# bwvdnbro/CMacIonize

Measured on AMD Instinct MI355X. Metric: photon packets/sec, 256^3 stromgren, higher is better.
Workload: dtype f64

## Files before the change

### cmacionize_amd/csrc/engine.hip

```cpp
#include "../../include/cmi_gpu.h"

#include "atomic_data.h"
#include "linecooling_data.h"
#include "kernels.h"
#include "dust_kernels.h"
#include "line_image_kernels.h"
#include "line_cube_kernels.h"
#include "sky_image_kernels.h"
#include "sky_cube_kernels.h"
#include "dust_cube_kernels.h"
#include "continuum_kernels.h"
#include "absorbing_cube_kernels.h"
#include "lyman_alpha_kernels.h"
#include "absorption_kernels.h"
#include "sort.h"

#include <algorithm>
#include <climits>
#include <cmath>
#include <cstdarg>
#include <cstdlib>
#include <cstdio>
#include <cstring>
#include <new>
// ... 102 lines not shown
  uint64_t tile_capacity = 0;
  bool tile_has_weights = false;
  FlightRowsDev tile_rows[2];
  uint32_t *tile_iota = nullptr;
  TileItemDev *tile_items = nullptr;
  uint32_t *tile_begin = nullptr;
  uint32_t *tile_blockhist = nullptr, *tile_total = nullptr;
  uint32_t *tile_new_slots = nullptr;
  TrackersDev trackers = {};
  bool trackers_enabled = false;
  EscapeDev escape = {};
  bool escape_counting = false;
  EscapeDev escape_staged = {};
  double *pad_H = nullptr;
  bool pad_valid = false;
  unsigned long long *metal_gate = nullptr;
  bool metals_pending = false;
  bool state_pointer_escaped = false;
  char *temp_pipe_block = nullptr;
  uint32_t temp_pipe_capacity = 0;
  unsigned int *temp_pipe_counts = nullptr;
  uint32_t *tile_ended_slot = nullptr;
  uint32_t *tile_ended_pos = nullptr;
  uint32_t *tile_slot_of[2] = {nullptr, nullptr};
  unsigned int *tile_absorbed_count = nullptr;
  unsigned int *tile_absorbed_before = nullptr;
  unsigned int *tile_counts = nullptr;
  uint64_t tile_rounds_run = 0;
  bool acc_block_dirty = false;

// ... 13 lines not shown
    bool reemit_passes = true;
    int refill_threshold_reemit = 32;
    int64_t reemit_inline_below = -1;
    int reemit_max_passes = 12;
    bool tile_rounds = true;
    uint64_t tile_min_flights = 100000;
    int tile_min_per_item = -1;
    int tile_refill_threshold = 48;
    bool tile_counting_sort = true;
    bool update_reuse = true;
    bool defer_metals = true;
    bool update_writes_pad = true;
    bool defer_weights = true;
    bool pre_emission = true;
    bool pad_march = true;
    bool xcd_remap = false;
    bool temperature_pipeline = true;
    uint32_t temperature_finish_slots = 1024;
    int tile_compact_ratio = -1;
    bool park_in_place = true;
    bool span_claim = CMI_SPAN_CLAIM_DEFAULT;
    bool emit_before_flush = CMI_EMIT_BEFORE_FLUSH_DEFAULT;
    bool phase_stamps = false;
    int continuum_channel_block = CMI_CONTINUUM_FB;
    int64_t continuum_launch_rays = 0;
    int absorbing_cube_channel_block = CMI_ABSORBING_CB;
    int absorbing_cube_expm1_call = CMI_ABSORBING_EXPM1_CALL;
    int absorbing_cube_window_skip = 1;
    int64_t absorbing_cube_launch_rays = 0;
    int absorption_slab_rows = 0;
// ... 606 lines not shown
  for (int64_t i = (int64_t)blockIdx.x * blockDim.x + threadIdx.x; i < n;
       i += step)
    dst[i * stride] = src[i];
}

int grid_blocks(cmi_gpu_engine *e, int64_t work_items, int blocks_per_cu) {
  int64_t want = (work_items + CMI_BLOCK - 1) / CMI_BLOCK;
  int64_t cap = (int64_t)e->num_cu * blocks_per_cu;
  if (want < 1)
    want = 1;
  return (int)(want < cap ? want : cap);
}

int update_full_flag(cmi_gpu_engine *e) {
  bool full = e->model.xsec_verner != 0;
  if (!full)
    for (int i = 1; i < CMI_NION; ++i)
      if (e->model.xsec_fixed[i] != 0.)
        full = true;
  if (full != e->full_ions)
    CMI_TRY(settle_metal_fractions(e));
  if (full != e->full_ions && e->acc_block) {
    if (hipSetDevice(e->device) != hipSuccess ||
        hipMemsetAsync(e->acc_block, 0,
                       (size_t)CMI_NACC * e->ncell * sizeof(double),
                       e->stream) != hipSuccess)
      e->acc_block_dirty = true;
  }
  e->full_ions = full;
  CellsDev &cells = cells_of_iteration(e);
// ... 724 lines not shown
  return field_pointer(e, field);
}

int cmi_gpu_get_update_state(cmi_gpu_engine *e, int32_t *metals_pending,
                             int32_t *pad_records_valid,
                             int32_t *deferral_allowed) {
  if (!e)
    return fail(CMI_GPU_EINVAL, "null engine");
  if (metals_pending)
    *metals_pending = e->metals_pending ? 1 : 0;
  if (pad_records_valid)
    *pad_records_valid = e->pad_valid ? 1 : 0;
  if (deferral_allowed)
    *deferral_allowed =
        (e->tune.defer_metals && !e->state_pointer_escaped) ? 1 : 0;
  return CMI_GPU_OK;
}

int cmi_gpu_reset_grid(cmi_gpu_engine *e) {
  if (!e)
    return fail(CMI_GPU_EINVAL, "null engine");
  HIP_TRY(hipSetDevice(e->device));
  const size_t field_bytes = (size_t)e->ncell * sizeof(double);
  if (e->full_ions || e->acc_block_dirty) {
    HIP_TRY(hipMemsetAsync(e->acc_block, 0, CMI_NACC * field_bytes,
                           e->stream));
    e->acc_block_dirty = false;
  } else {
    HIP_TRY(hipMemsetAsync(e->acc_block, 0, field_bytes, e->stream));
    if (e->config.track_heating)
// ... 55 lines not shown
  else if (k == "tile_refill_threshold")
    e->tune.tile_refill_threshold =
        (int)(value < 1 ? 1 : (value > 64 ? 64 : value));
  else if (k == "tile_compact_ratio")
    e->tune.tile_compact_ratio = (int)(value < -1 ? -1 : value);
  else if (k == "park_in_place")
    e->tune.park_in_place = value != 0;
  else if (k == "accumulators_dirty")
    e->acc_block_dirty = e->acc_block_dirty || value != 0;
  else if (k == "temperature_finish_slots")
    e->tune.temperature_finish_slots = (uint32_t)(value < 0 ? 0 : value);
  else if (k == "temperature_pipeline")
    e->tune.temperature_pipeline = value != 0;
  else if (k == "pad_march")
    e->tune.pad_march = value != 0;
  else if (k == "xcd_remap")
    e->tune.xcd_remap = value != 0;
  else if (k == "pre_emission")
    e->tune.pre_emission = value != 0;
  else if (k == "defer_weights")
    e->tune.defer_weights = value != 0;
  else if (k == "tile_counting_sort")
    e->tune.tile_counting_sort = value != 0;
  else if (k == "update_reuse")
    e->tune.update_reuse = value != 0;
  else if (k == "defer_metals")
    e->tune.defer_metals = value != 0;
  else if (k == "update_writes_pad")
    e->tune.update_writes_pad = value != 0;
  else if (k == "span_claim")
// ... 335 lines not shown
  const double volume =
      e->grid.cellside[0] * e->grid.cellside[1] * e->grid.cellside[2];
  a.jfac = jfac / volume;
  a.hfac = hfac / volume;
  a.first = first_cell;
  a.count = ncell;

  EventPair ev;
  CMI_TRY(timer_begin(e, ev));
  const int blocks = grid_blocks(e, ncell, 8);
  if (defer) {
    HydrogenUpdateArgs h;
    h.u = a;
    h.gate = e->metal_gate;
    h.pad_H = (e->pad_valid && e->tune.update_writes_pad) ? e->pad_H : nullptr;
    h.ny = (uint32_t)e->grid.ncell[1];
    h.nz = (uint32_t)e->grid.ncell[2];
    if (!h.pad_H)
      pad_records_stale(e);
    if (e->config.track_heating)
      hydrogen_update_kernel<true><<<blocks, CMI_BLOCK, 0, e->stream>>>(h);
    else
      hydrogen_update_kernel<false><<<blocks, CMI_BLOCK, 0, e->stream>>>(h);
    HIP_TRY(hipGetLastError());
    e->metals_pending = true;
    CMI_TRY(timer_end(e, e->update_events, ev, 0));
    return CMI_GPU_OK;
  }
  pad_records_stale(e);
  if (solve_temperature && e->tune.temperature_pipeline) {
// ... 736 lines not shown
```

### cmacionize_amd/csrc/kernels.h

```cpp
#ifndef CMI_KERNELS_H
#define CMI_KERNELS_H

#include "device_transport.h"
#include "device_reemit.h"
#include "device_thermal.h"
#include "device_emissivity.h"

#ifndef CMI_BLOCK
#define CMI_BLOCK 256
#endif
#ifdef CMI_EXPERIMENTS
#define CMI_EXP(a) ((a).exp_no_atomics)
#else
#define CMI_EXP(a) 0
#endif
#ifndef CMI_TABLE_BITS
#define CMI_TABLE_BITS 10
#endif
#define CMI_TABLE_SLOTS (1 << CMI_TABLE_BITS)
#ifndef CMI_TABLE_BLOCK
#define CMI_TABLE_BLOCK 512
#endif
#ifndef CMI_TABLE_BLOCK_BITS
#define CMI_TABLE_BLOCK_BITS 11
// ... 98 lines not shown
  uint32_t seed;
  uint32_t iteration;
  int32_t refill_threshold;
  int32_t exp_no_atomics;
  TrackersDev trackers;
  int32_t aggregate;
  QueueDev qin, qout;
  int32_t park_in_place;
  const double *xin;
  int32_t xin_local;
#ifdef CMI_DBG_XIN_SLOTS
  const uint32_t *xin_slots = nullptr;
#endif
  ExchangeDev xout;
  const double *pad_H;
  int32_t xcd_remap;
  int32_t pad_ny, pad_nz;
  double pad_inv_yz, pad_inv_z;
  uint32_t *span_cursor;
  uint32_t n_spans;
  int32_t span_claim;
  int32_t emit_before_flush;
#ifdef CMI_EXPERIMENTS
  unsigned long long *phase_clock;
#endif
};

#define CMI_SPAN_WANTED 0xfffffffeu
#define CMI_SPAN_NONE 0xffffffffu
#define CMI_SPAN_CURSORS 8
// ... 7 lines not shown
  CMI_PHASE_COUNT
};

#ifndef CMI_FULL_WAVES
#define CMI_FULL_WAVES 4
#endif
#ifndef CMI_PAD_WAVES
#define CMI_PAD_WAVES 8
#endif
#ifndef CMI_PAD_SCAN_ROUNDS
#define CMI_PAD_SCAN_ROUNDS 3
#endif
#define CMI_PAD_LAYERS 1
#define CMI_PAD_VACUUM (-0.)
#define CMI_PAD_GHOST (-2.)
__device__ __forceinline__ int32_t cmi_pad_index(int32_t offset) {
  return (int32_t)((uint32_t)offset >> 3);
}
__device__ __forceinline__ int32_t cmi_unpad_cell(const ShootArgs &a,
                                                  const GridDev &g,
                                                  int32_t c) {
  const double cc = (double)c + 0.5;
  const int32_t ix = (int32_t)(cc * a.pad_inv_yz);
  const int32_t r = c - ix * (a.pad_ny * a.pad_nz);
  const int32_t iy = (int32_t)(((double)r + 0.5) * a.pad_inv_z);
  const int32_t iz = r - iy * a.pad_nz;
  return ((ix - CMI_PAD_LAYERS) * g.ncell[1] + (iy - CMI_PAD_LAYERS)) *
             g.ncell[2] +
         (iz - CMI_PAD_LAYERS);
}
// ... 594 lines not shown
    const int32_t gi = p.index[ax] + g.offset[ax];
    in_block &= (p.index[ax] >= 0 && p.index[ax] < g.ncell[ax]);
    in_grid &= (gi >= 0 && gi < g.global_ncell[ax]);
  }
  const bool at_origin = (g.offset[0] | g.offset[1] | g.offset[2]) == 0;
  bool mine = in_block || (!in_grid && at_origin);
  if (g.copy_count > 1)
    mine &= (int32_t)(packet_id % (uint32_t)g.copy_count) == g.copy_rank;
  return mine;
}

#ifndef CMI_FULL_PASS_WAVES
#define CMI_FULL_PASS_WAVES 3
#endif
template <bool FULL, bool HEAT, bool REEMIT, bool EXACT, bool TABLE = false,
          bool PRE = false, bool PAD = false, bool TRACK = false,
          bool BIG = false>
__global__ void
    __launch_bounds__((shoot_block_threads<FULL, TABLE, BIG>()),
                      REEMIT ? 1
                             : (FULL ? (TABLE ? CMI_FULL_WAVES
                                              : CMI_FULL_PASS_WAVES)
                                    : ((PAD && !HEAT) ? CMI_PAD_WAVES
                                       : BIG          ? 4
                                                      : 6)))
        shoot_kernel(const ShootArgs a) {
  static_assert(!BIG || PAD, "BIG: the padded march on large grids");
  constexpr int BLOCK = shoot_block_threads<FULL, TABLE, BIG>();
  constexpr int TBITS =
      (TABLE && !FULL)
          ? (BIG ? CMI_TABLE_BLOCK_BIG_BITS : CMI_TABLE_BLOCK_BITS)
          : CMI_TABLE_BITS;
  constexpr int TSLOTS = 1 << TBITS;
  static_assert(!PAD || (TABLE && !FULL && !REEMIT && !EXACT && !PRE),
                "PAD is a specialisation of the hydrogen-only TABLE kernel");
  static_assert(!TRACK || (!TABLE && !EXACT && !PRE && !PAD),
                "TRACK is the tracker hook in the plain incremental marcher");
  const int lane = threadIdx.x & 63;
  const uint64_t lane_lt = (1ull << lane) - 1ull;
  uint32_t block = blockIdx.x;
  if (a.xcd_remap) {
    const uint32_t xcd = block & 7u, q = gridDim.x >> 3, r = gridDim.x & 7u;
    block = (xcd < r ? xcd * (q + 1u) : r * (q + 1u) + (xcd - r) * q) +
            (block >> 3);
  }
  const uint64_t wave = (uint64_t)block * (BLOCK / 64) +
                        (threadIdx.x >> 6);
  const uint64_t nwaves = (uint64_t)gridDim.x * (BLOCK / 64);
  const uint64_t chunk = a.chunk;

  uint64_t chunk_begin = wave * chunk;
  uint64_t pos = chunk_begin;
// ... 142 lines not shown
            atomic_add_f64(a.cells.acc_base + (int64_t)t * CMI_NACC + i,
                           lds_val[k * CMI_NACC + i]);
            lds_val[k * CMI_NACC + i] = 0.;
            ++natomics;
          }
          if (i == 0)
            lds_tag[k] = -1;
        }
      }
    } else {
      for (int k = threadIdx.x; k < lds_slots; k += BLOCK) {
        const int32_t t = lds_tag[TS * k];
        if (PAD ? t != -1 : t >= 0) {
          const int32_t c =
              PAD ? cmi_unpad_cell(a, a.grid, cmi_pad_index(t)) : t;
          atomic_add_f64(acc_at(a.cells, ION_H_n, c), lds_val[k]);
          lds_val[k] = 0.;
          if (HEAT) {
            atomic_add_f64(acc_at(a.cells, CMI_NION, c),
                           lds_val[lds_slots + k]);
            lds_val[lds_slots + k] = 0.;
          }
          lds_tag[TS * k] = -1;
          natomics += HEAT ? 2 : 1;
        }
      }
    }
    int any_work = 0, all_waves = 2;
#pragma unroll
    for (int w = 0; w < BLOCK / 64; ++w) {
      any_work |= block_has_work[w];
// ... 68 lines not shown
      }
      if (lanes_of(found)) {
        atomicAdd(&lds_val[slot], v0);
        if (HEAT)
          atomicAdd(&lds_val[TSLOTS + slot], v1);
      }
      looking &= ~found;
      if (lanes_of(looking))
        slot = (slot + 1) & (TSLOTS - 1);
      if (looking == 0ull)
        return;
    }
    if (lanes_of(looking)) {
      const int32_t c =
          PAD ? cmi_unpad_cell(a, a.grid, cmi_pad_index(cell)) : cell;
      atomic_add_f64(acc_at(a.cells, ION_H_n, c), v0);
      if (HEAT)
        atomic_add_f64(acc_at(a.cells, CMI_NION, c), v1);
      natomics += HEAT ? 2 : 1;
    }
  };
  for (;;) {
    const unsigned long long active_mask = __ballot(active);
    const unsigned long long idle_mask = ~active_mask;
    if (!claim && pos == pos_end &&
        chunk_begin + nwaves * chunk < a.n_packets) {
      chunk_begin += nwaves * chunk;
      pos = chunk_begin;
      pos_end = chunk_begin + chunk < a.n_packets ? chunk_begin + chunk
                                                  : a.n_packets;
    }
// ... 147 lines not shown
      }
      const uint64_t taken = __popcll(idle_mask);
      pos += taken < avail ? taken : avail;
    }
    CMI_PHASE_MARK(CMI_PHASE_REFILL);
    if (CLAIM && refill_first && !flush_point(has_work))
      break;
    const uint64_t avail_after =
        (pos_end - pos) +
        (!claim && chunk_begin + nwaves * chunk < a.n_packets ? 1 : 0);

    int window = 0;
    if (FULL)
      load_quarter_weights(stage, wq);
    if constexpr (PAD) {
      const double sigma = p.sigma_H;
      double wsig = p.weight * p.sigma_H;
      double hw = HEAT ? wsig * (p.nu - a.model.nu_H) : 0.;
      asm volatile("" : "+v"(wsig), "+v"(hw));
      const unsigned long long active_lanes = wave_ballot(active);
      int32_t not_lane = ~(lane << 3);
      asm volatile("" : "+v"(not_lane));
      const __attribute__((address_space(1))) char *pad_base =
          (const __attribute__((address_space(1))) char *)a.pad_H;
      asm volatile("" : "+s"(pad_base));
      const int idle_limit = __builtin_amdgcn_readfirstlane(
          avail_after != 0 ? a.refill_threshold : 65);
      const int fly_min = idle_limit < 64 ? 64 - idle_limit : 0;
      int zero = 0;
      asm volatile("" : "+v"(zero));
      const RunMasks pad_run_masks = run_masks<CMI_PAD_SCAN_ROUNDS>();
      unsigned int bundle_steps = 0;
      unsigned int bundle_lane_steps = 0;
      unsigned long long in_flight = active_lanes & mask_gt(p.tau, 0.);
      unsigned long long flying = in_flight & mask_gt(pad_next, -1.5);
      int nflying = (int)__popcll(flying);
      if (nflying > fly_min) do {
        ++bundle_steps;
        bundle_lane_steps += (unsigned int)nflying;
        const bool stepping = lanes_of(flying);
        const unsigned long long accumulating =
            flying & mask_ge(__double2hiint(pad_next), 0);
        int32_t key = lanes_of(accumulating) ? p.cell : not_lane;
        asm volatile("" : "+v"(key));
        double ds;
        asm volatile("" : "=v"(ds));
        if (stepping) {
          const double tmin =
              min_f64(p.tmax[0], min_f64(p.tmax[1], p.tmax[2]));
          const double t_old = p.t;
          ds = tmin - t_old;
          const double sk = sigma * pad_next;
          p.tau -= ds * sk;
          {
            unsigned long long saved;
            asm volatile("s_and_saveexec_b64 %[saved], %[m0]\n\t"
                         "v_add_f64 %[t0], %[t0], %[d0]\n\t"
                         "v_add_u32 %[cell], %[cell], %[c0]\n\t"
                         "s_and_b64 exec, %[saved], %[m1]\n\t"
                         "v_add_f64 %[t1], %[t1], %[d1]\n\t"
                         "v_add_u32 %[cell], %[cell], %[c1]\n\t"
                         "s_and_b64 exec, %[saved], %[m2]\n\t"
                         "v_add_f64 %[t2], %[t2], %[d2]\n\t"
                         "v_add_u32 %[cell], %[cell], %[c2]\n\t"
                         "s_mov_b64 exec, %[saved]"
                         : [t0] "+v"(p.tmax[0]), [t1] "+v"(p.tmax[1]),
                           [t2] "+v"(p.tmax[2]), [cell] "+v"(p.cell),
// ... 15 lines not shown
              double corr = p.tau * r;
              corr = __fma_rn(__fma_rn(-corr, sk, p.tau), r, corr);
              ds += corr;
              p.t = t_old + ds;
            }
          }
          pad_next = *reinterpret_cast<
              const __attribute__((address_space(1))) double *>(
              pad_base + (uint32_t)p.cell);
        }
        in_flight = flying & mask_gt(p.tau, 0.);
        if (CMI_EXP(a) == 12) {
          asm volatile("" ::"v"(ds), "s"(accumulating));
          continue;
        }
        double v[2] = {ds * wsig, HEAT ? ds * hw : 0.};
        unsigned long long tails;
        if (HEAT)
          run_sums_masked<2, CMI_PAD_SCAN_ROUNDS>(key, v, tails, zero,
                                                  pad_run_masks);
        else
          run_sums_masked<1, CMI_PAD_SCAN_ROUNDS>(
              key, reinterpret_cast<double(&)[1]>(v), tails, zero,
              pad_run_masks);
        if (CMI_EXP(a) == 11) {
          asm volatile("" ::"v"(v[0]), "s"(tails));
          continue;
        }
        table_add_masked(tails & accumulating, key, v[0], v[1]);
      } while ((flying = in_flight & mask_gt(pad_next, -1.5),
                nflying = (int)__popcll(flying), nflying > fly_min));
// ... 1297 lines not shown
      if (use_stored) {
        const MetalTermsStored terms = {&stored};
        ionization_update_cell<HEATING>(a, c, ntot, T, J, heating, terms);
      } else {
        const MetalTermsEvaluated terms = {a.model, T, T * 1.e-4};
        ionization_update_cell<HEATING>(a, c, ntot, T, J, heating, terms);
      }
    }
  }
}

struct HydrogenUpdateArgs {
  UpdateArgs u;
  unsigned long long *gate;
  double *pad_H;
  uint32_t ny, nz;
};

#ifndef CMI_HYDROGEN_UPDATE_WAVES
#define CMI_HYDROGEN_UPDATE_WAVES 4
#endif
template <bool HEATING>
__global__ void __launch_bounds__(CMI_BLOCK, CMI_HYDROGEN_UPDATE_WAVES)
    hydrogen_update_kernel(const HydrogenUpdateArgs h) {
  constexpr int WAVES = CMI_BLOCK / 64;
  const UpdateArgs &a = h.u;
  const int64_t rows = (a.count + 63) >> 6;
  const int64_t nwaves = (int64_t)gridDim.x * WAVES;
  const uint32_t lane = threadIdx.x & 63u;
  for (int64_t row = (int64_t)blockIdx.x * WAVES + (threadIdx.x >> 6);
// ... 15 lines not shown
      a.cells.x[ION_He_n][c] = he0;
      if (HEATING) {
        (*acc_at(a.cells, CMI_NION, c)) = heating[0];
        (*acc_at(a.cells, CMI_NION + 1, c)) = heating[1];
      }
      const double2 k = (ntot > 0.) ? make_double2(ntot * h0, ntot * he0)
                                    : make_double2(-1., 0.);
      a.cells.opacity[c] = k;
      if (h.pad_H) {
        constexpr uint32_t L = CMI_PAD_LAYERS;
        const uint32_t cc = (uint32_t)c;
        const uint32_t xy = cc / h.nz, pz = cc - xy * h.nz;
        const uint32_t px = xy / h.ny, py = xy - px * h.ny;
        const uint32_t padded =
            ((px + L) * (h.ny + 2 * L) + (py + L)) * (h.nz + 2 * L) + pz + L;
        h.pad_H[padded] = (k.x >= 0.) ? k.x : CMI_PAD_VACUUM;
      }
    }
    const unsigned long long word = wave_ballot(gate);
    if (lane == 0)
      h.gate[row] = word;
  }
}

struct MetalFractionsArgs {
  ModelDev model;
  CellsDev cells;
  int64_t count;
  const unsigned long long *gate;
};

// ... 277 lines not shown
__global__ void __launch_bounds__(CMI_BLOCK)
    opacity_kernel(const CellsDev cells, int64_t ncell) {
  const int64_t stride = (int64_t)gridDim.x * blockDim.x;
  for (int64_t c = (int64_t)blockIdx.x * blockDim.x + threadIdx.x; c < ncell;
       c += stride) {
    const double ntot = cells.number_density[c];
    cells.opacity[c] =
        (ntot > 0.) ? make_double2(ntot * cells.x[ION_H_n][c],
                                   ntot * cells.x[ION_He_n][c])
                    : make_double2(-1., 0.);
  }
}

__global__ void __launch_bounds__(CMI_BLOCK)
    pad_record_kernel(const double2 *__restrict__ opacity, double *pad,
                      int32_t nx, int32_t ny, int32_t nz) {
  const int64_t total = (int64_t)(nx + 2 * CMI_PAD_LAYERS) *
                        (ny + 2 * CMI_PAD_LAYERS) * (nz + 2 * CMI_PAD_LAYERS);
  const int64_t stride = (int64_t)gridDim.x * blockDim.x;
  for (int64_t c = (int64_t)blockIdx.x * blockDim.x + threadIdx.x; c < total;
       c += stride) {
    constexpr int L = CMI_PAD_LAYERS;
    const int32_t pz = (int32_t)(c % (nz + 2 * L)) - L;
    const int32_t py = (int32_t)((c / (nz + 2 * L)) % (ny + 2 * L)) - L;
    const int32_t px = (int32_t)(c / ((int64_t)(nz + 2 * L) * (ny + 2 * L))) - L;
    double v = CMI_PAD_GHOST;
    if (px >= 0 && px < nx && py >= 0 && py < ny && pz >= 0 && pz < nz) {
      const double k = opacity[((int64_t)px * ny + py) * nz + pz].x;
      v = (k >= 0.) ? k : CMI_PAD_VACUUM;
    }
    pad[c] = v;
  }
}


__global__ void emit_probe_kernel(const GridDev grid, const ModelDev model,
                                  uint32_t seed, uint32_t iteration,
                                  uint64_t first, uint64_t n, double *position,
                                  double *direction, double *frequency,
                                  double *sigma, double *tau) {
  const uint64_t i = (uint64_t)blockIdx.x * blockDim.x + threadIdx.x;
  if (i >= n)
    return;
  PacketRng rng;
  rng.init(seed, iteration, first + i);
// ... 72 lines not shown
```

### cmacionize_amd/csrc/transport_driver.h

```cpp
#ifndef CMI_TRANSPORT_DRIVER_H
#define CMI_TRANSPORT_DRIVER_H

static int reserve_sort_buffers(cmi_gpu_engine *e, uint64_t n) {
  if (e->sort_capacity >= n)
    return CMI_GPU_OK;
  HIP_TRY(hipStreamSynchronize(e->stream));
  (void)hipFree(e->sort_keys[0]);
  (void)hipFree(e->sort_temp);
  e->sort_keys[0] = nullptr;
  e->sort_temp = nullptr;
  e->sort_capacity = 0;
  uint32_t *block = nullptr;
  HIP_TRY(hipMalloc(&block, sizeof(uint32_t) * 4 * n));
  e->sort_keys[0] = block;
  e->sort_keys[1] = block + n;
  e->sort_ids[0] = block + 2 * n;
  e->sort_ids[1] = block + 3 * n;
  size_t bytes = 0;
  HIP_TRY(cmi_sort_pairs_temp_bytes(n, 32, &bytes));
  e->sort_temp_bytes = bytes;
  HIP_TRY(hipMalloc(&e->sort_temp, bytes ? bytes : 16));
  e->sort_capacity = n;
  return CMI_GPU_OK;
}
// ... 169 lines not shown
  FIRST_PAD_BIG,
  FIRST_PRE
};

struct LaunchPlan {
  bool heat, reemit;
  bool exact;
  bool tracking;
  bool passes;
  bool tiles;
  bool sorted;
  bool select_mode;
  int agg, agg_reemit;
  FirstBuild first;
  bool pad, pad_big;
  int64_t padded_cells;
  ShootKernel kernel, kernel_inline, kernel_first;
  int blocks_per_cu, blocks_per_cu_inline, blocks_per_cu_first;
  int first_threads;
  uint32_t tau_bits, source_bits, dir_bits;
  int key_bits;
  double sigma_ref;
  TileKernel tile_kernel;
  int tile_threads, tile_blocks_per_cu;
};

static ShootKernel shoot_build(bool full, bool heat, bool reemit, bool exact,
                               bool track, FirstBuild first) {
  static const ShootKernel generic[2][4][2] = {
      {{shoot_kernel<false, false, false, false>,
        shoot_kernel<false, false, true, false>},
       {shoot_kernel<false, true, false, false>,
        shoot_kernel<false, true, true, false>},
       {shoot_kernel<true, false, false, false>,
        shoot_kernel<true, false, true, false>},
       {shoot_kernel<true, true, false, false>,
        shoot_kernel<true, true, true, false>}},
      {{shoot_kernel<false, false, false, true>,
        shoot_kernel<false, false, true, true>},
       {shoot_kernel<false, true, false, true>,
        shoot_kernel<false, true, true, true>},
       {shoot_kernel<true, false, false, true>,
        shoot_kernel<true, false, true, true>},
// ... 1 lines not shown
        shoot_kernel<true, true, true, true>}}};
  static const ShootKernel tracked[4][2] = {
      {shoot_kernel<false, false, false, false, false, false, false, true>,
       shoot_kernel<false, false, true, false, false, false, false, true>},
      {shoot_kernel<false, true, false, false, false, false, false, true>,
       shoot_kernel<false, true, true, false, false, false, false, true>},
      {shoot_kernel<true, false, false, false, false, false, false, true>,
       shoot_kernel<true, false, true, false, false, false, false, true>},
      {shoot_kernel<true, true, false, false, false, false, false, true>,
       shoot_kernel<true, true, true, false, false, false, false, true>}};
  static const ShootKernel table[2][2] = {
      {shoot_kernel<true, true, false, false, true>,
       shoot_kernel<true, false, false, false, true>},
      {shoot_kernel<false, true, false, false, true>,
       shoot_kernel<false, false, false, false, true>}};
  static const ShootKernel pad_big[2] = {
      shoot_kernel<false, true, false, false, true, false, true, false, true>,
      shoot_kernel<false, false, false, false, true, false, true, false, true>};
  static const ShootKernel pad[2] = {
      shoot_kernel<false, true, false, false, true, false, true>,
      shoot_kernel<false, false, false, false, true, false, true>};
  static const ShootKernel pre[2] = {
      shoot_kernel<true, true, false, false, true, true>,
      shoot_kernel<true, false, false, false, true, true>};
  switch (first) {
  case FIRST_TABLE:
    return table[!full][!heat];
  case FIRST_PAD:
    return pad[!heat];
  case FIRST_PAD_BIG:
    return pad_big[!heat];
  case FIRST_PRE:
    return pre[!heat];
  case FIRST_GENERIC:
    break;
  }
  return track ? tracked[2 * full + heat][reemit]
               : generic[exact][2 * full + heat][reemit];
}

extern "C++" {
template <class Kernel>
static int blocks_per_cu_of(Kernel kernel, int threads, int most, int &out) {
  out = 0;
  HIP_TRY(hipOccupancyMaxActiveBlocksPerMultiprocessor(&out, kernel, threads,
                                                       0));
// ... 18 lines not shown
  p.exact = tune.exact_dda || !small_grid ||
            (p.tracking && !e->grid.decomposed);
  p.passes = p.reemit && tune.reemit_passes &&
             !(flights && n_packets < reemit_inline_below(e));
  p.sorted = tune.sort_packets && !flights;
  p.tiles = p.passes && tune.tile_rounds && !p.exact && !p.tracking;
  p.select_mode = p.sorted && e->grid.decomposed;

  const bool table =
      !flights && !p.exact && !p.tracking && p.agg == CMI_AGG_BLOCK &&
      (p.passes || !p.reemit) &&
      !(e->grid.periodic[0] | e->grid.periodic[1] | e->grid.periodic[2]);
  p.padded_cells = ((int64_t)e->grid.ncell[0] + 2 * CMI_PAD_LAYERS) *
                   ((int64_t)e->grid.ncell[1] + 2 * CMI_PAD_LAYERS) *
                   ((int64_t)e->grid.ncell[2] + 2 * CMI_PAD_LAYERS);
  p.pad = table && !e->full_ions && tune.pad_march &&
          p.padded_cells < ((int64_t)1 << 29);
  p.pad_big = p.pad && e->ncell > CMI_TABLE_BIG_CELLS;
  p.first = FIRST_GENERIC;
  if (p.pad)
    p.first = p.pad_big ? FIRST_PAD_BIG : FIRST_PAD;
  else if (table && e->full_ions && tune.pre_emission && p.sorted &&
           p.tiles)
    p.first = FIRST_PRE;
  else if (table)
    p.first = FIRST_TABLE;
  p.first_threads = (table && !e->full_ions)
                        ? (p.pad_big ? shoot_block_threads<false, true, true>()
                                     : shoot_block_threads<false, true>())
                        : CMI_BLOCK;

  const bool track = p.tracking && !p.exact;
  p.kernel_inline =
      shoot_build(e->full_ions, p.heat, true, p.exact, track, FIRST_GENERIC);
  p.kernel = (p.reemit && !p.passes)
                 ? p.kernel_inline
                 : shoot_build(e->full_ions, p.heat, false, p.exact, track,
                               FIRST_GENERIC);
  p.kernel_first = table ? shoot_build(e->full_ions, p.heat, false, false,
                                       false, p.first)
                         : p.kernel;
  CMI_TRY(blocks_per_cu_of(p.kernel, CMI_BLOCK, tune.max_blocks_per_cu,
                           p.blocks_per_cu));
  CMI_TRY(blocks_per_cu_of(p.kernel_inline, CMI_BLOCK, tune.max_blocks_per_cu,
                           p.blocks_per_cu_inline));
  p.blocks_per_cu_first = p.blocks_per_cu;
  if (table)
    CMI_TRY(blocks_per_cu_of(p.kernel_first, p.first_threads,
                             tune.max_blocks_per_cu, p.blocks_per_cu_first));
  p.tile_kernel = nullptr;
  p.tile_threads = p.tile_blocks_per_cu = 0;
  if (p.tiles) {
    if (e->full_ions)
      p.tile_kernel =
          p.heat ? tile_kernel<true, true> : tile_kernel<true, false>;
// ... 98 lines not shown
  a.grid = e->grid;
  a.model = e->model;
  a.cells = cells_of_iteration(e);
  a.counters = e->counters;
  a.first_packet = first_packet;
  a.batch_offset = done;
  a.n_packets = nids;
  a.order = nullptr;
  a.pre_rows = nullptr;
  a.xin = flights ? flights + (size_t)CMI_FLIGHT_DOUBLES * done : nullptr;
  a.xin_local = 0;
  a.xout.rows = e->export_rows;
  a.xout.count = e->export_count;
  a.xout.capacity = (unsigned int)e->export_capacity;
  a.pad_H = p.pad ? e->pad_H : nullptr;
  a.xcd_remap = (p.sorted && e->tune.xcd_remap) ? 1 : 0;
  a.pad_ny = e->grid.ncell[1] + 2 * CMI_PAD_LAYERS;
  a.pad_nz = e->grid.ncell[2] + 2 * CMI_PAD_LAYERS;
  a.pad_inv_yz = 1. / ((double)a.pad_ny * (double)a.pad_nz);
  a.pad_inv_z = 1. / (double)a.pad_nz;
  a.chunk = e->tune.chunk;
  a.seed = seed;
  a.iteration = iteration;
  a.refill_threshold = flights ? e->tune.refill_threshold_reemit
                               : e->tune.refill_threshold;
  a.exp_no_atomics = e->tune.exp_no_atomics;
  a.trackers = e->trackers;
  if (!p.tracking)
    a.trackers.n = 0;
  a.aggregate = flights ? p.agg_reemit : p.agg;
// ... 6 lines not shown
  a.emit_before_flush = e->tune.emit_before_flush ? 1 : 0;
#ifdef CMI_EXPERIMENTS
  a.phase_clock = nullptr;
#endif
  return a;
}

static int pad_records(cmi_gpu_engine *e, const LaunchPlan &p) {
  if (e->pad_valid)
    return CMI_GPU_OK;
  const GridDev &g = e->grid;
  if (!e->pad_H)
    HIP_TRY(hipMalloc(&e->pad_H, sizeof(double) * (size_t)p.padded_cells));
  pad_record_kernel<<<grid_blocks(e, p.padded_cells, 8), CMI_BLOCK, 0,
                      e->stream>>>(cells_of_iteration(e).opacity, e->pad_H,
                                   g.ncell[0], g.ncell[1], g.ncell[2]);
  HIP_TRY(hipGetLastError());
  e->pad_valid = true;
  return CMI_GPU_OK;
}

static int select_block_packets(cmi_gpu_engine *e, ShootArgs &a,
                                const uint32_t **select) {
  const uint64_t nids = a.n_packets;
  if (!e->select_count)
    HIP_TRY(hipMalloc(&e->select_count, sizeof(unsigned int)));
  CMI_TRY(grow(e, e->select_ids, e->select_capacity, nids,
               sizeof(uint32_t) * nids));
  HIP_TRY(hipMemsetAsync(e->select_count, 0, sizeof(unsigned int),
                         e->stream));
  SelectArgs sa;
// ... 477 lines not shown
                "cmi_gpu_shoot: at most 2^32 - 2 packets per call");
  if (e->grid.decomposed &&
      (e->tune.exact_dda || !e->export_rows ||
       e->ncell >= CMI_FAST_MARCHER_MAX_CELLS))
    return fail(CMI_GPU_ESTATE,
                "cmi_gpu_shoot: a block of a decomposed grid needs an export "
                "buffer (cmi_gpu_set_export_buffer) and the incremental "
                "marcher (fewer than 2^28 cells per block)");
  if (!flights && e->grid.decomposed && block_emits_nothing(e))
    return CMI_GPU_OK;
  HIP_TRY(hipSetDevice(e->device));
  CMI_TRY(ensure_spectra(e));

  LaunchPlan plan;
  CMI_TRY(plan_launches(e, n_packets, flights, plan));
  CMI_TRY(publish_escape(e, plan.tracking));
  const uint64_t max_launch = e->tune.max_packets_per_launch;
  if (!plan.select_mode)
    CMI_TRY(reserve_for(e, plan, n_packets < max_launch ? n_packets
                                                         : max_launch));
  if (plan.pad)
    CMI_TRY(pad_records(e, plan));

  for (uint64_t done = 0; done < n_packets; done += max_launch) {
    const uint64_t nids = n_packets - done < max_launch ? n_packets - done
                                                        : max_launch;
    ShootArgs a = shoot_args(e, plan, seed, iteration, first_packet, done,
                             nids, flights);
    const uint32_t *select = nullptr;
    if (plan.select_mode) {
// ... 25 lines not shown
```

### cmacionize_amd/engine.py

```python
import ctypes as C
import os

import numpy as np

_HERE = os.path.dirname(os.path.abspath(__file__))
LIB_PATH = os.environ.get("CMI_GPU_LIBRARY",
                          os.path.join(_HERE, "libcmi_gpu.so"))

NION = 14
TRACKER_SPECTRUM, TRACKER_ABSORPTION, TRACKER_WEIGHTED_SPECTRUM = 0, 1, 2
NACC = 16
NTYPE = 4

FIELD_NUMBER_DENSITY = 0
FIELD_TEMPERATURE = 1
FIELD_IONIC_FRACTION = 2
FIELD_MEAN_INTENSITY = 16
FIELD_HEATING = 30

REEMIT_NONE, REEMIT_PHYSICAL, REEMIT_FIXED = 0, 1, 2
CONTINUOUS_NONE, CONTINUOUS_ISOTROPIC, CONTINUOUS_PLANAR = 0, 1, 2
ROLE_SOURCE, ROLE_CONTINUOUS = 0, 1
TABLE_LINEAR, TABLE_LOGLOG = 0, 1
DUST_PROBE_EMIT, DUST_PROBE_SCATTER, DUST_PROBE_SCATTER_TOWARDS = 0, 1, 2
# ... 100 lines not shown
    "cmi_gpu_render_continuum_sky_map", "cmi_gpu_continuum_probe",
    "cmi_gpu_hi_coefficients", "cmi_gpu_render_hi_cube",
    "cmi_gpu_render_hi_sky_cube", "cmi_gpu_render_hi_sky_map_cube",
    "cmi_gpu_render_field_absorbing_cube",
    "cmi_gpu_render_field_absorbing_sky_cube",
    "cmi_gpu_absorbing_cube_probe", "cmi_gpu_get_update_state",
    "cmi_gpu_set_lyman_alpha", "cmi_gpu_lya_shoot", "cmi_gpu_lya_probe",
    "cmi_gpu_download_lya_view", "cmi_gpu_reset_lya",
    "cmi_gpu_get_lya_counters", "cmi_gpu_lyman_alpha_emissivity",
    "cmi_gpu_set_lya_field", "cmi_gpu_download_lya_field",
    "cmi_gpu_lya_spin_temperature",
    "cmi_gpu_render_field_absorption_spectra",
    "cmi_gpu_render_absorption_spectra", "cmi_gpu_absorption_probe",
    "cmi_gpu_set_escape_tally", "cmi_gpu_reset_escape_tally",
    "cmi_gpu_download_escape_tally", "cmi_gpu_escape_pixels",
    "cmi_gpu_cross_sections",
]

EMISSION_LINES = [
    "HAlpha", "HBeta", "HII", "BALMER_JUMP_LOW", "BALMER_JUMP_HIGH",
    "OI_6300", "OI_6364", "OII_3727", "OIII_5007", "OIII_4959", "OIII_4363",
    "OIII_52mu", "OIII_88mu", "NII_5755", "NII_6548", "NII_6584",
    "NeIII_3869", "NeIII_3968", "SII_6725", "SII_4072", "SIII_9405",
    "SIII_6312", "SIII_19mu", "SIII_33mu", "avg_T", "avg_T_count",
    "avg_nH_nHe", "avg_nH_nHe_count", "NeII_12mu", "NIII_57mu", "NeIII_15mu",
    "NII_122mu", "CII_158mu", "CII_2325", "CIII_1908", "OII_7325", "SIV_10mu",
    "HeI_5876", "Hrec_s", "WFC2_F439W", "WFC2_F555W", "WFC2_F675W"]

_ELEMENT_WEIGHTS = {"H": 1.00794, "He": 4.002602, "C": 12.0107, "N": 14.0067,
                    "O": 15.9994, "Ne": 20.1797, "S": 32.065}

# ... 131 lines not shown
    L.cmi_gpu_set_cross_sections_verner.argtypes = [vp]
    L.cmi_gpu_set_recombination_rates_fixed.argtypes = [vp, _dp]
    L.cmi_gpu_set_recombination_rates_verner.argtypes = [vp]
    L.cmi_gpu_set_abundances.argtypes = [vp, _dp]
    L.cmi_gpu_set_reemission.argtypes = [vp, C.c_int32, C.c_double,
                                         C.c_double]
    L.cmi_gpu_set_temperature_params.argtypes = [
        vp, C.POINTER(TemperatureParams)]
    L.cmi_gpu_upload_cells.argtypes = [vp, _dp, _dp, _dp]
    L.cmi_gpu_upload_field.argtypes = [vp, C.c_int32, _dp]
    L.cmi_gpu_download_field.argtypes = [vp, C.c_int32, _dp]
    L.cmi_gpu_field_device_pointer.restype = C.c_void_p
    L.cmi_gpu_field_device_pointer.argtypes = [vp, C.c_int32]
    if hasattr(L, "cmi_gpu_get_update_state"):
        L.cmi_gpu_get_update_state.argtypes = [vp] + 3 * [C.POINTER(C.c_int32)]
    L.cmi_gpu_reset_grid.argtypes = [vp]
    L.cmi_gpu_shoot.argtypes = [vp, C.c_uint32, C.c_uint32, C.c_uint64,
                                C.c_uint64]
    L.cmi_gpu_get_counters.argtypes = [vp, _dp, _dp, C.POINTER(C.c_uint64)]
    L.cmi_gpu_update_cells.argtypes = [vp, C.c_uint32, C.c_double]
    L.cmi_gpu_emit_packets.argtypes = [vp, C.c_uint32, C.c_uint32, C.c_uint64,
                                       C.c_uint64, _dp, _dp, _dp, _dp, _dp]
    L.cmi_gpu_trace_packets.argtypes = [
        vp, C.c_uint64, _dp, _dp, _dp, _dp, _dp, C.c_int32,
        C.POINTER(C.c_int64), _dp, C.POINTER(C.c_int32), C.POINTER(C.c_int64),
        _dp]
    L.cmi_gpu_get_timing.argtypes = [vp, C.c_int32, _dp, C.POINTER(C.c_uint64),
                                     _dp, C.POINTER(C.c_uint64)]
    L.cmi_gpu_get_kernel_timing.argtypes = [vp, _dp, C.POINTER(C.c_uint64)]
    L.cmi_gpu_set_tuning.argtypes = [vp, C.c_char_p, C.c_int64]
# ... 582 lines not shown
    def accumulator_layout(self):
        fs, cs = C.c_int64(), C.c_int64()
        self._check(self._lib.cmi_gpu_accumulator_layout(
            self._h, C.byref(fs), C.byref(cs)))
        return fs.value, cs.value

    def field_device_pointer(self, field):
        return self._lib.cmi_gpu_field_device_pointer(self._h, field)

    def update_state(self):
        v = [C.c_int32() for _ in range(3)]
        self._check(self._lib.cmi_gpu_get_update_state(
            self._h, *[C.byref(x) for x in v]))
        return tuple(bool(x.value) for x in v)

    def field_tensor(self, field):
        import torch
        ptr = self.field_device_pointer(field)
        n = self.n

        class _View:
            __cuda_array_interface__ = {
                "shape": (n,), "typestr": "<f8", "data": (int(ptr), False),
                "version": 2}
        return torch.as_tensor(_View(), device="cuda")

    def refresh_transport_records(self):
        self._check(self._lib.cmi_gpu_refresh_transport_records(self._h))

    def reset_grid(self):
# ... 1186 lines not shown
```

### include/cmi_gpu.h

```cpp
#ifndef CMI_GPU_H
#define CMI_GPU_H

#include <stddef.h>
#include <stdint.h>

#ifdef __cplusplus
extern "C" {
#endif

#define CMI_GPU_NION 14
#define CMI_GPU_NHEATING 2
#define CMI_GPU_NTYPE 4
#define CMI_GPU_NACC (CMI_GPU_NION + CMI_GPU_NHEATING)

enum {
  CMI_GPU_OK = 0,
  CMI_GPU_EINVAL = 1,
  CMI_GPU_EDEVICE = 2,
  CMI_GPU_ESTATE = 3,
  CMI_GPU_ENOMEM = 4
};

enum {
  CMI_GPU_FIELD_NUMBER_DENSITY = 0,
// ... 102 lines not shown
int cmi_gpu_set_temperature_params(cmi_gpu_engine *engine,
                                   const cmi_gpu_temperature_params *params);


int cmi_gpu_upload_cells(cmi_gpu_engine *engine, const double *number_density,
                         const double *temperature,
                         const double *ionic_fractions);
int cmi_gpu_upload_field(cmi_gpu_engine *engine, int32_t field,
                         const double *values);
int cmi_gpu_download_field(cmi_gpu_engine *engine, int32_t field,
                           double *values);
void *cmi_gpu_field_device_pointer(cmi_gpu_engine *engine, int32_t field);
int cmi_gpu_get_update_state(cmi_gpu_engine *engine, int32_t *metals_pending,
                             int32_t *pad_records_valid,
                             int32_t *deferral_allowed);
int cmi_gpu_accumulator_layout(cmi_gpu_engine *engine, int64_t *field_stride,
                               int64_t *cell_stride);


int cmi_gpu_reset_grid(cmi_gpu_engine *engine);

int cmi_gpu_shoot(cmi_gpu_engine *engine, uint32_t seed, uint32_t iteration,
                  uint64_t first_packet, uint64_t n_packets);

#define CMI_GPU_FLIGHT_DOUBLES 16
int cmi_gpu_set_export_buffer(cmi_gpu_engine *engine, void *device_rows,
                              uint64_t capacity);
int cmi_gpu_get_export_count(cmi_gpu_engine *engine, uint64_t *count);
int cmi_gpu_reset_exports(cmi_gpu_engine *engine);
int cmi_gpu_download_exports(cmi_gpu_engine *engine, double *host_rows,
// ... 480 lines not shown
```

Measured before the change: 4.005 billion.

## Pre-multiply hydrogen cross-section into pad records and add uniform-weight PAD kernel

Pad records now store sigma_H times opacity, so the marcher's per-step multiply by sigma goes away. When packet weights are uniform and heating is off, a new specialised PAD kernel accumulates raw path lengths and applies a single weight times sigma scale at the atomic flush, removing a per-packet multiply and a register. Pad validity is now reset whenever the cross-section setup may change. The change also adds a query API reporting the chosen plan, and it rounds products differently than before.

```diff
diff --git a/cmacionize_amd/csrc/engine.hip b/cmacionize_amd/csrc/engine.hip
--- a/cmacionize_amd/csrc/engine.hip
+++ b/cmacionize_amd/csrc/engine.hip
@@ -140,6 +140,8 @@
   EscapeDev escape_staged = {};
   double *pad_H = nullptr;
   bool pad_valid = false;
+  int32_t last_first_build = 0;
+  bool last_pad_uniform = false;
   unsigned long long *metal_gate = nullptr;
   bool metals_pending = false;
   bool state_pointer_escaped = false;
@@ -183,6 +185,7 @@
     bool defer_weights = true;
     bool pre_emission = true;
     bool pad_march = true;
+    bool pad_uniform = true;
     bool xcd_remap = false;
     bool temperature_pipeline = true;
     uint32_t temperature_finish_slots = 1024;
@@ -819,6 +822,7 @@
 
 int update_full_flag(cmi_gpu_engine *e) {
   bool full = e->model.xsec_verner != 0;
+  e->pad_valid = false;
   if (!full)
     for (int i = 1; i < CMI_NION; ++i)
       if (e->model.xsec_fixed[i] != 0.)
@@ -1573,6 +1577,17 @@
   if (deferral_allowed)
     *deferral_allowed =
         (e->tune.defer_metals && !e->state_pointer_escaped) ? 1 : 0;
+  return CMI_GPU_OK;
+}
+
+int cmi_gpu_get_transport_plan(cmi_gpu_engine *e, int32_t *first_build,
+                               int32_t *uniform_weight) {
+  if (!e)
+    return fail(CMI_GPU_EINVAL, "null engine");
+  if (first_build)
+    *first_build = e->last_first_build;
+  if (uniform_weight)
+    *uniform_weight = e->last_pad_uniform ? 1 : 0;
   return CMI_GPU_OK;
 }
 
@@ -1658,6 +1673,8 @@
     e->tune.temperature_pipeline = value != 0;
   else if (k == "pad_march")
     e->tune.pad_march = value != 0;
+  else if (k == "pad_uniform")
+    e->tune.pad_uniform = value != 0;
   else if (k == "xcd_remap")
     e->tune.xcd_remap = value != 0;
   else if (k == "pre_emission")
@@ -2023,6 +2040,7 @@
     h.u = a;
     h.gate = e->metal_gate;
     h.pad_H = (e->pad_valid && e->tune.update_writes_pad) ? e->pad_H : nullptr;
+    h.pad_sigma = e->model.xsec_fixed[ION_H_n];
     h.ny = (uint32_t)e->grid.ncell[1];
     h.nz = (uint32_t)e->grid.ncell[2];
     if (!h.pad_H)
diff --git a/cmacionize_amd/csrc/kernels.h b/cmacionize_amd/csrc/kernels.h
--- a/cmacionize_amd/csrc/kernels.h
+++ b/cmacionize_amd/csrc/kernels.h
@@ -136,6 +136,7 @@
 #endif
   ExchangeDev xout;
   const double *pad_H;
+  double uniform_scale;
   int32_t xcd_remap;
   int32_t pad_ny, pad_nz;
   double pad_inv_yz, pad_inv_z;
@@ -173,6 +174,9 @@
 #define CMI_PAD_LAYERS 1
 #define CMI_PAD_VACUUM (-0.)
 #define CMI_PAD_GHOST (-2.)
+__device__ __forceinline__ double cmi_pad_record(double sigma, double nx) {
+  return sigma * ((nx >= 0.) ? nx : CMI_PAD_VACUUM);
+}
 __device__ __forceinline__ int32_t cmi_pad_index(int32_t offset) {
   return (int32_t)((uint32_t)offset >> 3);
 }
@@ -797,7 +801,7 @@
 #define CMI_FULL_PASS_WAVES 3
 #endif
 template <bool FULL, bool HEAT, bool REEMIT, bool EXACT, bool TABLE = false,
-          bool PRE = false, bool PAD = false, bool TRACK = false,
+          bool PRE = false, bool PAD = false, bool SWITCH8 = false,
           bool BIG = false>
 __global__ void
     __launch_bounds__((shoot_block_threads<FULL, TABLE, BIG>()),
@@ -817,8 +821,12 @@
   constexpr int TSLOTS = 1 << TBITS;
   static_assert(!PAD || (TABLE && !FULL && !REEMIT && !EXACT && !PRE),
                 "PAD is a specialisation of the hydrogen-only TABLE kernel");
-  static_assert(!TRACK || (!TABLE && !EXACT && !PRE && !PAD),
+  constexpr bool TRACK = SWITCH8 && !PAD;
+  static_assert(!TRACK || (!TABLE && !EXACT && !PRE),
                 "TRACK is the tracker hook in the plain incremental marcher");
+  constexpr bool UNIFORM = SWITCH8 && PAD;
+  static_assert(!UNIFORM || !HEAT,
+                "the heating term's weight differs from packet to packet");
   const int lane = threadIdx.x & 63;
   const uint64_t lane_lt = (1ull << lane) - 1ull;
   uint32_t block = blockIdx.x;
@@ -991,7 +999,8 @@
         if (PAD ? t != -1 : t >= 0) {
           const int32_t c =
               PAD ? cmi_unpad_cell(a, a.grid, cmi_pad_index(t)) : t;
-          atomic_add_f64(acc_at(a.cells, ION_H_n, c), lds_val[k]);
+          atomic_add_f64(acc_at(a.cells, ION_H_n, c),
+                         UNIFORM ? lds_val[k] * a.uniform_scale : lds_val[k]);
           lds_val[k] = 0.;
           if (HEAT) {
             atomic_add_f64(acc_at(a.cells, CMI_NION, c),
@@ -1090,7 +1099,8 @@
     if (lanes_of(looking)) {
       const int32_t c =
           PAD ? cmi_unpad_cell(a, a.grid, cmi_pad_index(cell)) : cell;
-      atomic_add_f64(acc_at(a.cells, ION_H_n, c), v0);
+      atomic_add_f64(acc_at(a.cells, ION_H_n, c),
+                     UNIFORM ? v0 * a.uniform_scale : v0);
       if (HEAT)
         atomic_add_f64(acc_at(a.cells, CMI_NION, c), v1);
       natomics += HEAT ? 2 : 1;
@@ -1268,10 +1278,10 @@
     if (FULL)
       load_quarter_weights(stage, wq);
     if constexpr (PAD) {
-      const double sigma = p.sigma_H;
-      double wsig = p.weight * p.sigma_H;
+      double wsig = UNIFORM ? 0. : p.weight * p.sigma_H;
       double hw = HEAT ? wsig * (p.nu - a.model.nu_H) : 0.;
-      asm volatile("" : "+v"(wsig), "+v"(hw));
+      if (!UNIFORM)
+        asm volatile("" : "+v"(wsig), "+v"(hw));
       const unsigned long long active_lanes = wave_ballot(active);
       int32_t not_lane = ~(lane << 3);
       asm volatile("" : "+v"(not_lane));
@@ -1295,16 +1305,16 @@
         const bool stepping = lanes_of(flying);
         const unsigned long long accumulating =
             flying & mask_ge(__double2hiint(pad_next), 0);
+        double t12 = min_f64(p.tmax[1], p.tmax[2]);
         int32_t key = lanes_of(accumulating) ? p.cell : not_lane;
-        asm volatile("" : "+v"(key));
+        asm volatile("" : "+v"(key), "+v"(t12));
         double ds;
         asm volatile("" : "=v"(ds));
         if (stepping) {
-          const double tmin =
-              min_f64(p.tmax[0], min_f64(p.tmax[1], p.tmax[2]));
+          const double tmin = min_f64(p.tmax[0], t12);
           const double t_old = p.t;
           ds = tmin - t_old;
-          const double sk = sigma * pad_next;
+          const double sk = pad_next;
           p.tau -= ds * sk;
           {
             unsigned long long saved;
@@ -1350,7 +1360,7 @@
           asm volatile("" ::"v"(ds), "s"(accumulating));
           continue;
         }
-        double v[2] = {ds * wsig, HEAT ? ds * hw : 0.};
+        double v[2] = {UNIFORM ? ds : ds * wsig, HEAT ? ds * hw : 0.};
         unsigned long long tails;
         if (HEAT)
           run_sums_masked<2, CMI_PAD_SCAN_ROUNDS>(key, v, tails, zero,
@@ -2678,6 +2688,7 @@
   UpdateArgs u;
   unsigned long long *gate;
   double *pad_H;
+  double pad_sigma;
   uint32_t ny, nz;
 };
 
@@ -2723,7 +2734,7 @@
         const uint32_t px = xy / h.ny, py = xy - px * h.ny;
         const uint32_t padded =
             ((px + L) * (h.ny + 2 * L) + (py + L)) * (h.nz + 2 * L) + pz + L;
-        h.pad_H[padded] = (k.x >= 0.) ? k.x : CMI_PAD_VACUUM;
+        h.pad_H[padded] = cmi_pad_record(h.pad_sigma, k.x);
       }
     }
     const unsigned long long word = wave_ballot(gate);
@@ -3031,7 +3042,7 @@
 
 __global__ void __launch_bounds__(CMI_BLOCK)
     pad_record_kernel(const double2 *__restrict__ opacity, double *pad,
-                      int32_t nx, int32_t ny, int32_t nz) {
+                      double sigma, int32_t nx, int32_t ny, int32_t nz) {
   const int64_t total = (int64_t)(nx + 2 * CMI_PAD_LAYERS) *
                         (ny + 2 * CMI_PAD_LAYERS) * (nz + 2 * CMI_PAD_LAYERS);
   const int64_t stride = (int64_t)gridDim.x * blockDim.x;
@@ -3042,10 +3053,9 @@
     const int32_t py = (int32_t)((c / (nz + 2 * L)) % (ny + 2 * L)) - L;
     const int32_t px = (int32_t)(c / ((int64_t)(nz + 2 * L) * (ny + 2 * L))) - L;
     double v = CMI_PAD_GHOST;
-    if (px >= 0 && px < nx && py >= 0 && py < ny && pz >= 0 && pz < nz) {
-      const double k = opacity[((int64_t)px * ny + py) * nz + pz].x;
-      v = (k >= 0.) ? k : CMI_PAD_VACUUM;
-    }
+    if (px >= 0 && px < nx && py >= 0 && py < ny && pz >= 0 && pz < nz)
+      v = cmi_pad_record(sigma,
+                         opacity[((int64_t)px * ny + py) * nz + pz].x);
     pad[c] = v;
   }
 }
diff --git a/cmacionize_amd/csrc/transport_driver.h b/cmacionize_amd/csrc/transport_driver.h
--- a/cmacionize_amd/csrc/transport_driver.h
+++ b/cmacionize_amd/csrc/transport_driver.h
@@ -207,6 +207,8 @@
   int agg, agg_reemit;
   FirstBuild first;
   bool pad, pad_big;
+  bool pad_uniform;
+  double uniform_scale;
   int64_t padded_cells;
   ShootKernel kernel, kernel_inline, kernel_first;
   int blocks_per_cu, blocks_per_cu_inline, blocks_per_cu_first;
@@ -219,7 +221,8 @@
 };
 
 static ShootKernel shoot_build(bool full, bool heat, bool reemit, bool exact,
-                               bool track, FirstBuild first) {
+                               bool track, FirstBuild first,
+                               bool uniform = false) {
   static const ShootKernel generic[2][4][2] = {
       {{shoot_kernel<false, false, false, false>,
         shoot_kernel<false, false, true, false>},
@@ -251,12 +254,14 @@
        shoot_kernel<true, false, false, false, true>},
       {shoot_kernel<false, true, false, false, true>,
        shoot_kernel<false, false, false, false, true>}};
-  static const ShootKernel pad_big[2] = {
+  static const ShootKernel pad_big[3] = {
       shoot_kernel<false, true, false, false, true, false, true, false, true>,
-      shoot_kernel<false, false, false, false, true, false, true, false, true>};
-  static const ShootKernel pad[2] = {
+      shoot_kernel<false, false, false, false, true, false, true, false, true>,
+      shoot_kernel<false, false, false, false, true, false, true, true, true>};
+  static const ShootKernel pad[3] = {
       shoot_kernel<false, true, false, false, true, false, true>,
-      shoot_kernel<false, false, false, false, true, false, true>};
+      shoot_kernel<false, false, false, false, true, false, true>,
+      shoot_kernel<false, false, false, false, true, false, true, true>};
   static const ShootKernel pre[2] = {
       shoot_kernel<true, true, false, false, true, true>,
       shoot_kernel<true, false, false, false, true, true>};
@@ -264,9 +269,9 @@
   case FIRST_TABLE:
     return table[!full][!heat];
   case FIRST_PAD:
-    return pad[!heat];
+    return pad[!heat + (!heat && uniform)];
   case FIRST_PAD_BIG:
-    return pad_big[!heat];
+    return pad_big[!heat + (!heat && uniform)];
   case FIRST_PRE:
     return pre[!heat];
   case FIRST_GENERIC:
@@ -315,9 +320,16 @@
   p.padded_cells = ((int64_t)e->grid.ncell[0] + 2 * CMI_PAD_LAYERS) *
                    ((int64_t)e->grid.ncell[1] + 2 * CMI_PAD_LAYERS) *
                    ((int64_t)e->grid.ncell[2] + 2 * CMI_PAD_LAYERS);
+  const double sigma_H = e->model.xsec_fixed[ION_H_n];
   p.pad = table && !e->full_ions && tune.pad_march &&
-          p.padded_cells < ((int64_t)1 << 29);
+          p.padded_cells < ((int64_t)1 << 29) && sigma_H >= 0. &&
+          std::isfinite(sigma_H);
   p.pad_big = p.pad && e->ncell > CMI_TABLE_BIG_CELLS;
+  const double pc = e->model.continuous_probability;
+  const double *pw = e->model.photon_weight;
+  p.pad_uniform = p.pad && !p.heat && tune.pad_uniform &&
+                  (pc <= 0. || pc >= 1. || pw[0] == pw[1]);
+  p.uniform_scale = (pc >= 1. ? pw[1] : pw[0]) * sigma_H;
   p.first = FIRST_GENERIC;
   if (p.pad)
     p.first = p.pad_big ? FIRST_PAD_BIG : FIRST_PAD;
@@ -339,7 +351,7 @@
                  : shoot_build(e->full_ions, p.heat, false, p.exact, track,
                                FIRST_GENERIC);
   p.kernel_first = table ? shoot_build(e->full_ions, p.heat, false, false,
-                                       false, p.first)
+                                       false, p.first, p.pad_uniform)
                          : p.kernel;
   CMI_TRY(blocks_per_cu_of(p.kernel, CMI_BLOCK, tune.max_blocks_per_cu,
                            p.blocks_per_cu));
@@ -468,6 +480,7 @@
   a.xout.count = e->export_count;
   a.xout.capacity = (unsigned int)e->export_capacity;
   a.pad_H = p.pad ? e->pad_H : nullptr;
+  a.uniform_scale = p.uniform_scale;
   a.xcd_remap = (p.sorted && e->tune.xcd_remap) ? 1 : 0;
   a.pad_ny = e->grid.ncell[1] + 2 * CMI_PAD_LAYERS;
   a.pad_nz = e->grid.ncell[2] + 2 * CMI_PAD_LAYERS;
@@ -504,7 +517,8 @@
     HIP_TRY(hipMalloc(&e->pad_H, sizeof(double) * (size_t)p.padded_cells));
   pad_record_kernel<<<grid_blocks(e, p.padded_cells, 8), CMI_BLOCK, 0,
                       e->stream>>>(cells_of_iteration(e).opacity, e->pad_H,
-                                   g.ncell[0], g.ncell[1], g.ncell[2]);
+                                   e->model.xsec_fixed[ION_H_n], g.ncell[0],
+                                   g.ncell[1], g.ncell[2]);
   HIP_TRY(hipGetLastError());
   e->pad_valid = true;
   return CMI_GPU_OK;
@@ -1012,6 +1026,10 @@
 
   LaunchPlan plan;
   CMI_TRY(plan_launches(e, n_packets, flights, plan));
+  if (!flights) {
+    e->last_first_build = (int32_t)plan.first;
+    e->last_pad_uniform = plan.pad_uniform;
+  }
   CMI_TRY(publish_escape(e, plan.tracking));
   const uint64_t max_launch = e->tune.max_packets_per_launch;
   if (!plan.select_mode)
diff --git a/cmacionize_amd/engine.py b/cmacionize_amd/engine.py
--- a/cmacionize_amd/engine.py
+++ b/cmacionize_amd/engine.py
@@ -138,7 +138,7 @@
     "cmi_gpu_render_absorption_spectra", "cmi_gpu_absorption_probe",
     "cmi_gpu_set_escape_tally", "cmi_gpu_reset_escape_tally",
     "cmi_gpu_download_escape_tally", "cmi_gpu_escape_pixels",
-    "cmi_gpu_cross_sections",
+    "cmi_gpu_cross_sections", "cmi_gpu_get_transport_plan",
 ]
 
 EMISSION_LINES = [
@@ -300,6 +300,9 @@
     L.cmi_gpu_field_device_pointer.argtypes = [vp, C.c_int32]
     if hasattr(L, "cmi_gpu_get_update_state"):
         L.cmi_gpu_get_update_state.argtypes = [vp] + 3 * [C.POINTER(C.c_int32)]
+    if hasattr(L, "cmi_gpu_get_transport_plan"):
+        L.cmi_gpu_get_transport_plan.argtypes = [vp] + 2 * [
+            C.POINTER(C.c_int32)]
     L.cmi_gpu_reset_grid.argtypes = [vp]
     L.cmi_gpu_shoot.argtypes = [vp, C.c_uint32, C.c_uint32, C.c_uint64,
                                 C.c_uint64]
@@ -912,6 +915,12 @@
             self._h, *[C.byref(x) for x in v]))
         return tuple(bool(x.value) for x in v)
 
+    def transport_plan(self):
+        first, uniform = C.c_int32(), C.c_int32()
+        self._check(self._lib.cmi_gpu_get_transport_plan(
+            self._h, C.byref(first), C.byref(uniform)))
+        return first.value, bool(uniform.value)
+
     def field_tensor(self, field):
         import torch
         ptr = self.field_device_pointer(field)
diff --git a/include/cmi_gpu.h b/include/cmi_gpu.h
--- a/include/cmi_gpu.h
+++ b/include/cmi_gpu.h
@@ -140,6 +140,8 @@
 int cmi_gpu_get_update_state(cmi_gpu_engine *engine, int32_t *metals_pending,
                              int32_t *pad_records_valid,
                              int32_t *deferral_allowed);
+int cmi_gpu_get_transport_plan(cmi_gpu_engine *engine, int32_t *first_build,
+                               int32_t *uniform_weight);
 int cmi_gpu_accumulator_layout(cmi_gpu_engine *engine, int64_t *field_stride,
                                int64_t *cell_stride);
 
```

New measurement: 4.107 billion (median of 6 runs). +2.5%, better.
